# korentomas/mlx-mcmc

Hardware: AMD Instinct MI355X
Metric: leapfrog-steps/sec (all chains) + ESS/sec, 1000-dim Gaussian @1/2/4/8 GPUs (higher is better)
Workload: dtype f32

## Files before the change

### mlx-mcmc_amd/csrc/lanes_fast_nc.h

```cpp
#pragma once
#include "lanes_fast.h"

namespace mc {

template <int NC>
using lf_vec = float __attribute__((ext_vector_type(NC)));
typedef lf_vec<1> f1;
MC_DEV f1 vpin(f1 x) {
    x[0] = vpin((float)x[0]);
    return x;
}
template <int NC>
MC_DEV lf_vec<NC> lf_mk(float a, float b) {
    if constexpr (NC == 2) return (f2){a, b};
    else return (f1){a};
}
template <int NC>
MC_DEV lf_vec<NC> lf_bc(float x) {
    return lf_mk<NC>(x, x);
}
template <class V>
MC_DEV V lf_fma(V a, V b, V c) { return __builtin_elementwise_fma(a, b, c); }
template <int NC>
MC_DEV lf_vec<NC> lf_shc(float v, int k) {
    lf_vec<NC> r;
#pragma unroll
    for (int c = 0; c < NC; ++c) r[c] = rl(v, lf_shlane(k, c));
    return r;
}

template <class V>
struct LfMomV {
    V c, R, R2, Q, n;
};
template <class V>
MC_DEV void lf_moments(const LfMomV<V>& m, V th, V& M1, V& M2) {
    const V d = m.c - th;
    M1 = lf_fma(m.n, d, m.R);
    M2 = lf_fma(lf_fma(m.n, d, m.R2), d, m.Q);
}

constexpr int lfc_draw_jobs(int D, int NC) { return NC * ((D + 3) / 4) + NC; }
constexpr LfDrawJob lfc_draw_job(int t, int D, int NC) {
    const int NBk = (D + 3) / 4;
    const bool acc = t >= NC * NBk;
    const int c = acc ? t - NC * NBk : (t >= NBk ? 1 : 0);
    return {acc, c, acc ? 0 : t - (c ? NBk : 0)};
}
constexpr bool lfc_draw_jobs_once(int D, int lanes, int NC) {
    const int NBk = (D + 3) / 4;
    int mom[2][257] = {}, acc[2] = {};
    if (NBk > 257) return false;
    for (int tid = 0; tid < lanes; ++tid)
        for (int t = tid; t < lfc_draw_jobs(D, NC); t += lanes) {
            const LfDrawJob jb = lfc_draw_job(t, D, NC);
            if (jb.c < 0 || jb.c >= NC || jb.b < 0 || jb.b >= NBk) return false;
            if (jb.acc) ++acc[jb.c];
            else ++mom[jb.c][jb.b];
        }
    for (int c = 0; c < NC; ++c) {
        if (acc[c] != 1) return false;
        for (int b = 0; b < NBk; ++b)
            if (mom[c][b] != 1) return false;
    }
    return true;
}
static_assert(lfc_draw_jobs(1000, 2) == lf_draw_jobs(1000) && lfc_draw_jobs_once(1000, 512, 2) &&
              lfc_draw_job(300, 1000, 2).c == lf_draw_job(300, 1000).c &&
              lfc_draw_job(501, 1000, 2).acc && lf_draw_job(501, 1000).acc,
              "NC = 2: the pair kernel's job map");
static_assert(lfc_draw_jobs(1000, 1) == 251 && lfc_draw_jobs_once(1000, 512, 1) &&
              lfc_draw_jobs_once(1027, 256, 1) && lfc_draw_jobs_once(5, 256, 1) &&
              lfc_draw_jobs_once(303, 256, 1) && lfc_draw_jobs_once(1024, 512, 1),
              "one chain's jobs");

template <int RS, int NSH, int NW, bool X1, int FORM, bool XL = false, int SPEC = 0, int DN = 0,
          int NC = 2>
__global__ void __launch_bounds__(64 * NW)
k_hmc_lfc(LrCtx P, RunArgs A, int64_t chain_base, int64_t n_groups, mc_chain_scalars* scal,
         float* st_q, float* st_g, float* samples, TraceDev tr, unsigned long long* xch,
         int* status, uint32_t ebase) {
    static_assert(NSH <= kLrMaxShared, "shared parameters");
    constexpr bool CF = FORM >= 0;
    static_assert(!CF || lf_nroles(FORM) == NSH, "record slots of a compile-time form");
    constexpr bool DENSE = DN > 0;
    static_assert(!DENSE || (DN == NW && DN >= 2 && DN <= kLrSlices && !X1 && !XL),
                  "dense: wave w is slice w, records through LDS");
    static_assert(DENSE && (NC == 1 || NC == 2), "k_hmc_lfc: the dense launches");
    typedef lf_vec<NC> fc;
    constexpr int NB = DENSE ? NC : 2 * NW;
    constexpr int NV = 2 * (NSH + 1);
    constexpr int NPAIR = NV + 4;
    constexpr int NPASS = (NPAIR + 3) / 4, NPASS_V = (NV + 3) / 4;
    constexpr int NRS = (NV + 7) / 8;
    if (!X1 && !DENSE && A.fault && blockIdx.x == gridDim.x - 1)
        return;
    extern __shared__ __attribute__((aligned(16))) float smem[];
    const mc_run_config& cfg = A.cfg;
    const int tid = threadIdx.x;
    const int wave = tid >> 6, j = tid & 63;
    const int S = DENSE ? DN : P.S, D = P.D, Dsh = P.Dsh;
    int64_t grp;
    int slice;
    if constexpr (DENSE) {
        grp = blockIdx.x;
        slice = wave;
    } else {
        const int64_t w = blockIdx.x, nwg = gridDim.x;
        if (nwg % 8 == 0 && (nwg / 8) % S == 0) {
            const int64_t x = w & 7, r = w >> 3;
            grp = x * ((nwg / 8) / S) + r / S;
            slice = (int)(r % S);
        } else {
            grp = w / S;
            slice = (int)(w % S);
        }
    }
    const int64_t C = cfg.num_chains;
    const int64_t cbase = chain_base + grp * NB;
    const int b0 = DENSE ? 0 : 2 * wave;
    int64_t cc[2];
    bool live[2];
#pragma unroll
    for (int c = 0; c < 2; ++c) {
        live[c] = c < NC && cbase + b0 + c < C;
        cc[c] = min(cbase + b0 + (c < NC ? c : 0), C - 1);
    }

    float* const xl = smem;
    const int64_t* blk = P.blocks + 4 * (int64_t)slice;
    const float* gd = P.data + blk[0];
    const int nsweep = (int)(blk[3] & 255);
    const int ndirect = (int)((blk[3] >> 8) & 255);
    LrSterm* sst = (LrSterm*)(smem + (DENSE ? 2 * DN * 16 : 0));
    for (int i = tid; i < P.n_sterms * (int)(sizeof(LrSterm) / 16); i += 64 * NW)
        ((float4*)sst)[i] = ((const float4*)P.sterms)[i];

    const MC_CONST LrTerm* tt = cptr(P.terms) + (int64_t)slice * P.n_terms;
    const LfTerms F = lf_terms(tt, nsweep, ndirect);
    const bool SW = CF ? (FORM & LF_SW) != 0 : F.sw;
    const bool SWS = CF ? (FORM & LF_SWS) != 0 : F.sw_shs;
    const bool DIR = CF ? (FORM & LF_DIR) != 0 : F.dir;
    const bool DM = CF ? (FORM & LF_DM) != 0 : F.d_shm;
    const bool DS = CF ? (FORM & LF_DS) != 0 : F.d_shs;
    const int ksw = CF ? lf_slot_sws(FORM) : max(F.sw_ks, 0);
    const int kdm = CF ? lf_slot_dm(FORM) : max(F.d_km, 0);
    const int kds = CF ? lf_slot_ds(FORM) : max(F.d_ks, 0);
    const int nsl = CF ? NSH : Dsh;
    auto ord_of = [&](int k) {
        int o = F.d_ks;
        o = (DM && k == kdm) ? F.d_km : o;
        o = (SWS && k == ksw) ? F.sw_ks : o;
        return CF ? o : k;
    };
    int xk = -1, xc = 0;
#pragma unroll
    for (int k = 0; k < kLrMaxShared; ++k)
#pragma unroll
        for (int c = 0; c < NC; ++c)
            if (k < nsl && lf_shlane(k, c) == j) {
                xk = k;
                xc = c;
            }
    const bool xon = xk >= 0;
    const int xo = xon ? ord_of(xk) : 0;
    int xg = P.shl[0];
#pragma unroll
    for (int k = 1; k < kLrMaxShared; ++k) xg = (xo == k) ? P.shl[k] : xg;
    const int64_t xch_id = xc ? cc[1] : cc[0];
    const bool xlive = xon && (xc ? live[1] : live[0]);
    const int rep = (SPEC & LFS_REP1) ? 1 : P.rep;
    const bool lead = (j & (rep - 1)) == 0;
    const bool hxf = (SPEC & LFS_NOXF) ? false : P.has_xf != 0;
    int xxf = P.shxf[0];
    float xid = P.shid[0];
#pragma unroll
    for (int k = 1; k < kLrMaxShared; ++k) {
        xxf = (xo == k) ? P.shxf[k] : xxf;
        xid = (xo == k) ? P.shid[k] : xid;
    }
    xxf = xon ? xxf : MC_XF_NONE;
    xid = xon ? xid : 0.0f;

    LrPriv<RS> R0;
    int gk[RS];
    fc q[RS], p[RS], g[RS];
#pragma unroll
    for (int r = 0; r < RS; ++r) {
        gk[r] = P.gidx[((int64_t)slice * kLrMaxSlots + r) * 64 + j];
#pragma unroll
        for (int c = 0; c < 2; ++c) {
            R0.q[r][c] = gk[r] >= 0 ? st_q[cc[c] * D + gk[r]] : 0.0f;
            R0.g[r][c] = gk[r] >= 0 ? st_g[cc[c] * D + gk[r]] : 0.0f;
        }
        q[r] = lf_mk<NC>(R0.q[r][0], R0.q[r][1]);
        g[r] = lf_mk<NC>(R0.g[r][0], R0.g[r][1]);
        p[r] = lf_bc<NC>(0.0f);
    }
    const bool rngp = P.rng != nullptr;
    int4 rw = {0, 0, 0, 0};
    if (rngp) rw = P.rng[(int64_t)slice * 64 + j];
    const int racc0 = __builtin_amdgcn_readfirstlane((rw.w >> 8) & 63);
    const int racc1 = __builtin_amdgcn_readfirstlane((rw.w >> 14) & 63);
    int sh_src = 0;
    if (rngp) {
        const int target = (xc + 1) | ((xg >> 2) << 3);
        for (int i = 0; i < 64; ++i)
            sh_src = (__builtin_amdgcn_readlane(rw.x, i) == target) ? i : sh_src;
    }
    LrShared sh;
    sh.q = xon ? st_q[xch_id * D + xg] : 1.0f;
    sh.g = xon ? st_g[xch_id * D + xg] : 0.0f;
    sh.p = 0.0f;
    sh.v = hxf ? xf_apply(xxf, sh.q) : sh.q;
    sh.is = sh.iv = 1.0f;
    sh.lg = 0.0f;
    double eps[2];
    fc lp;
    int nacc[2], ntot[2], wacc[2], wtot[2];
#pragma unroll
    for (int c = 0; c < NC; ++c) {
        eps[c] = scal[cc[c]].step_size;
        lp[c] = scal[cc[c]].logp;
        nacc[c] = scal[cc[c]].n_accept;
        ntot[c] = scal[cc[c]].n_total;
        wacc[c] = scal[cc[c]].warmup_accept;
        wtot[c] = scal[cc[c]].warmup_total;
    }
    constexpr bool BDRAW = (DENSE || (X1 && RS == 4)) &&
                           FORM == (LF_SW | LF_SWS | LF_DIR | LF_DM | LF_DS) &&
                           SPEC == (LFS_REP1 | LFS_NOXF);
    const bool bdraw = BDRAW && P.blk_rng != 0;
    const int NBk = (D + 3) >> 2;
    const int ZB = 4 * NC * NBk + 4;
    static_assert(sizeof(LrSterm) % 16 == 0, "the draws' float4 stores follow the scalar terms");
    float* const zl = (float*)sst + P.n_sterms * (int)(sizeof(LrSterm) / 4);
    auto draw_block = [&](int64_t itd) {
        float* const zb = zl + (int)(itd & 1) * ZB;
        for (int t = tid; t < lfc_draw_jobs(D, NC); t += 64 * NW) {
            const LfDrawJob jb = lfc_draw_job(t, D, NC);
            const bool acl = jb.acc;
            const int c = jb.c, b = jb.b;
            const mc_u32x4 rr =
                mc_draw(cfg.seed, (uint32_t)(cfg.chain_offset + (c ? cc[1] : cc[0])),
                        (uint32_t)itd, acl ? MC_RNG_TAG_ACCEPT : MC_RNG_TAG_MOMENTUM, 0,
                        acl ? 0u : (uint32_t)b);
            const float la = mc_logf_unit(acl ? mc_u01_f32(rr.x) : mc_u01_boxf(rr.x));
            const float lb = mc_logf_unit(mc_u01_boxf(rr.z));
            float4 z;
            mc_box_muller_log(la, rr.y, &z.x, &z.y);
            mc_box_muller_log(lb, rr.w, &z.z, &z.w);
            if (acl) zb[4 * NC * NBk + c] = la;
            else *(float4*)(zb + 4 * (c * NBk + b)) = z;
        }
    };
    if constexpr (BDRAW) {
        if (bdraw && cfg.iter_count > 0) draw_block(cfg.iter_begin);
    }
    MC_STAMP_INIT
    __syncthreads();

    const LrOwn own = lr_own_prior(P.n_sterms, sst, xon ? 2 * xo + xc : 64, Dsh);
    const bool own_lp0 = own.on && slice == 0 && xc == 0;
    const bool own_lp1 = own.on && slice == 0 && xc == 1;
    const float o_m = vpin(own.hn ? 0.0f : own.m), o_cinv2 = vpin(own.cinv2),
                o_c0l = vpin(own.c0l), o_wn = vpin(own.wn);
    auto own_grad = [&](float v) {
        const float d = v - o_m;
        const bool out = own.hn && !(v >= 0.0f);
        return (out || !own.on) ? 0.0f : o_wn * -(d * o_cinv2);
    };
    int len[RS];
    fc cnt[RS];
    LfMomV<fc> mom[RS];
    bool pdir[RS];
#pragma unroll
    for (int r = 0; r < RS; ++r) {
        float4 m = {0.f, 0.f, 0.f, 0.f};
        if (SW && r < tt[0].nslot) m = P.mom[((int64_t)slice * kLrMaxSlots + r) * 64 + j];
        len[r] = (int)m.w;
        cnt[r] = lf_bc<NC>(m.w);
        mom[r].c = vpin(lf_bc<NC>(m.x));
        mom[r].R = vpin(lf_bc<NC>(m.y));
        mom[r].R2 = vpin(lf_bc<NC>(m.y + m.y));
        mom[r].Q = vpin(lf_bc<NC>(m.z));
        mom[r].n = cnt[r];
        pdir[r] = DIR && r < tt[nsweep].nslot &&
                  ((const int32_t*)gd)[tt[nsweep].len_off + r * 64 + j] > 0;
    }
    const fc sw_w = vpin(lf_bc<NC>(F.sw_w)), sw_c0 = vpin(lf_bc<NC>(F.sw_c0));
    const fc sw_cinv = vpin(lf_bc<NC>(F.sw_cinv)), sw_cinv2 = vpin(lf_bc<NC>(F.sw_cinv2)),
             sw_clogs = vpin(lf_bc<NC>(F.sw_clogs));
    const fc d_w = vpin(lf_bc<NC>(F.d_w)), d_c0 = vpin(lf_bc<NC>(F.d_c0)), d_m = vpin(lf_bc<NC>(F.d_m));
    const fc d_w1 = vpin(lf_bc<NC>(pdir[0] ? F.d_w : 0.0f));
    const fc d_cinv = vpin(lf_bc<NC>(F.d_cinv)), d_cinv2 = vpin(lf_bc<NC>(F.d_cinv2)),
             d_clogs = vpin(lf_bc<NC>(F.d_clogs));
    const fc half = lf_bc<NC>(0.5f), one = lf_bc<NC>(1.0f);
    const float lp_const = vpin(P.lp_const);
    const int L = cfg.num_leapfrog_steps;
    uint32_t epoch = ebase;
    bool ok = true;
    unsigned long long* gline[2];
#pragma unroll
    for (int par = 0; par < 2; ++par)
        gline[par] = DENSE ? nullptr
                           : xch + (((int64_t)par * n_groups + grp) * (NB / 2) + wave) * S * 16;
    const int row = j >> 4, col = j & 15;
    const bool poll_lane = col < S;
    unsigned long long* gp[2];
#pragma unroll
    for (int par = 0; par < 2; ++par)
        gp[par] = DENSE ? nullptr : gline[par] + min(col, S - 1) * 16 + lf_row(row);
    const int lpoll = min(col, S - 1) * 16 + lf_row(row);
    auto lput = [&](int par, int off, float v) { xl[par * (DN * 16) + off] = v; };
    const int pub_pair = (col < 2 * NRS) ? 8 * (col >> 1) + 4 * (col & 1) + lf_row(row) : -1;
    const bool pub_rec = pub_pair >= 0 && pub_pair < NV && (NC == 2 || !(pub_pair & 1));
    const bool pub_mid = pub_rec && pub_pair >= 2;
    const int pub_x = 2 * (col >> 1) + (col & 1);
    const int pub_off = slice * 16 + max(pub_pair, 0);
    uint32_t need_v = 0, need_lp = 0, need_k0 = 0, need_k1 = 0;
#pragma unroll
    for (int ps = 0; ps < NPASS; ++ps) {
        const int pr = 4 * ps + lf_row(row);
        if (X1 || !poll_lane || pr >= NPAIR || (NC == 1 && (pr & 1))) continue;
        if (pr < 2) need_lp |= 1u << ps;
        else if (pr < NV) need_v |= 1u << ps;
        else if (pr < NV + 2) need_k0 |= 1u << ps;
        else need_k1 |= 1u << ps;
    }
    constexpr bool xchk = XL && !X1;
    unsigned long long* const xslots = xch + ((int64_t)grp * (NB / 2)) * S * 16 + 15;
    XcdPoll xpoll = {0ull};
    if (xchk && cfg.iter_count > 0)
        xpoll = xcd_announce(xslots, S, slice, ebase + 1, wave == 0 && j == 0);
    static_assert(NPAIR <= 15, "granule 15 of a record line is the XCD handshake's");
    const int64_t it_end = cfg.iter_begin + cfg.iter_count;
    constexpr bool DRAW_AHEAD = RS == 1 && CF && (SPEC & LFS_REP1) != 0;
    fc nx_z[RS];
    float nx_sh = 0.0f, nx_lu[2] = {0.f, 0.f};
#pragma unroll
    for (int r = 0; r < RS; ++r) nx_z[r] = lf_bc<NC>(0.0f);
    auto draw_plan = [&](int64_t itd) {
        const int kind = rw.x & 7;
        const bool acl = kind >= 3;
        const int csel = (kind == 2 || kind == 4) ? 1 : 0;
        const mc_u32x4 rr =
            mc_draw(cfg.seed, (uint32_t)(cfg.chain_offset + (csel ? cc[1] : cc[0])),
                    (uint32_t)itd, acl ? MC_RNG_TAG_ACCEPT : MC_RNG_TAG_MOMENTUM, 0,
                    acl ? 0u : ((uint32_t)rw.x >> 3));
        const float la = mc_logf_unit(acl ? mc_u01_f32(rr.x) : mc_u01_boxf(rr.x));
        const float lb = mc_logf_unit(mc_u01_boxf(rr.z));
        float z[4];
        mc_box_muller_log(la, rr.y, &z[0], &z[1]);
        mc_box_muller_log(lb, rr.w, &z[2], &z[3]);
        nx_lu[0] = rl(la, racc0);
        nx_lu[1] = rl(la, racc1);
        auto fetch = [&](int src, int comp) {
            float v = __shfl(z[0], src);
            const float v1 = __shfl(z[1], src), v2 = __shfl(z[2], src), v3 = __shfl(z[3], src);
            v = comp == 1 ? v1 : v;
            v = comp == 2 ? v2 : v;
            return comp == 3 ? v3 : v;
        };
#pragma unroll
        for (int r = 0; r < RS; ++r) {
            const int word = (r < 2 ? rw.y : rw.z) >> (14 * (r & 1));
            const int comp = (word >> 12) & 3;
            nx_z[r] = lf_mk<NC>(fetch(word & 63, comp), fetch((word >> 6) & 63, comp));
        }
        nx_sh = fetch(sh_src, xg & 3);
    };
    if (DRAW_AHEAD && rngp && cfg.iter_count > 0) draw_plan(cfg.iter_begin);
    for (int64_t it = cfg.iter_begin; it < it_end && ok; ++it) {
        MC_STAMP_DECL
        const bool warm = it < cfg.num_warmup;
        float hs[2], es[2];
#pragma unroll
        for (int c = 0; c < NC; ++c) {
            if (it == cfg.num_warmup) {
                wacc[c] = nacc[c];
                wtot[c] = ntot[c];
                nacc[c] = 0;
                ntot[c] = 0;
            }
            hs[c] = (float)(0.5 * eps[c]);
            es[c] = (float)eps[c];
        }
        if constexpr (NC == 1) {
            hs[1] = hs[0];
            es[1] = es[0];
        }
        const fc h = vpin(lf_mk<NC>(hs[0], hs[1])), e = vpin(lf_mk<NC>(es[0], es[1]));
        const float xh = vpin(xc ? hs[1] : hs[0]), xe = vpin(xc ? es[1] : es[0]);
        auto normal_of = [&](int gi, int64_t chain) {
            const mc_u32x4 rr = mc_draw(cfg.seed, (uint32_t)(cfg.chain_offset + chain),
                                        (uint32_t)it, MC_RNG_TAG_MOMENTUM, 0, (uint32_t)(gi >> 2));
            float z0, z1;
            if ((gi & 3) < 2) mc_box_muller(rr.x, rr.y, &z0, &z1);
            else mc_box_muller(rr.z, rr.w, &z0, &z1);
            return (gi & 1) ? z1 : z0;
        };
        fc k0p = lf_bc<NC>(0.0f);
        float logu_acc[2] = {0.f, 0.f};
        if (rngp) {
            if constexpr (DRAW_AHEAD) {
                logu_acc[0] = nx_lu[0];
                logu_acc[1] = nx_lu[1];
#pragma unroll
                for (int r = 0; r < RS; ++r) {
                    if (gk[r] < 0) continue;
                    p[r] = nx_z[r];
                    if (lead) k0p += nx_z[r] * nx_z[r];
                }
                sh.p = xon ? nx_sh : 0.0f;
            } else {
                const int kind = rw.x & 7;
                const bool acl = kind >= 3;
                const int csel = (kind == 2 || kind == 4) ? 1 : 0;
                const mc_u32x4 rr =
                    mc_draw(cfg.seed, (uint32_t)(cfg.chain_offset + (csel ? cc[1] : cc[0])),
                            (uint32_t)it, acl ? MC_RNG_TAG_ACCEPT : MC_RNG_TAG_MOMENTUM, 0,
                            acl ? 0u : ((uint32_t)rw.x >> 3));
                const float la = mc_logf_unit(acl ? mc_u01_f32(rr.x) : mc_u01_boxf(rr.x));
                const float lb = mc_logf_unit(mc_u01_boxf(rr.z));
                float z[4];
                mc_box_muller_log(la, rr.y, &z[0], &z[1]);
                mc_box_muller_log(lb, rr.w, &z[2], &z[3]);
                logu_acc[0] = rl(la, racc0);
                logu_acc[1] = rl(la, racc1);
                auto fetch = [&](int src, int comp) {
                    float v = __shfl(z[0], src);
                    const float v1 = __shfl(z[1], src), v2 = __shfl(z[2], src), v3 = __shfl(z[3], src);
                    v = comp == 1 ? v1 : v;
                    v = comp == 2 ? v2 : v;
                    return comp == 3 ? v3 : v;
                };
    #pragma unroll
                for (int r = 0; r < RS; ++r) {
                    const int word = (r < 2 ? rw.y : rw.z) >> (14 * (r & 1));
                    const int comp = (word >> 12) & 3;
                    const fc zz = lf_mk<NC>(fetch(word & 63, comp), fetch((word >> 6) & 63, comp));
                    if (gk[r] < 0) continue;
                    p[r] = zz;
                    if (lead) k0p += zz * zz;
                }
                const float zs = fetch(sh_src, xg & 3);
                sh.p = xon ? zs : 0.0f;
            }
        } else if (bdraw) {
            if constexpr (X1) __syncthreads();
            const float* const zb = zl + (int)(it & 1) * ZB;
#pragma unroll
            for (int c = 0; c < NC; ++c) logu_acc[c] = zb[4 * NC * NBk + c];
#pragma unroll
            for (int r = 0; r < RS; ++r) {
                const int gi = max(gk[r], 0);
                fc z;
#pragma unroll
                for (int c = 0; c < NC; ++c) z[c] = zb[4 * NBk * c + gi];
                if (gk[r] >= 0) {
                    p[r] = z;
                    if (lead) k0p += z * z;
                }
            }
            const float zs = zb[(xc ? 4 * NBk : 0) + xg];
            sh.p = xon ? zs : 0.0f;
        } else {
#pragma unroll
            for (int r = 0; r < RS; ++r) {
                if (gk[r] < 0) continue;
                fc z;
#pragma unroll
                for (int c = 0; c < NC; ++c) z[c] = normal_of(gk[r], cc[c]);
                p[r] = z;
                if (lead) k0p += z * z;
            }
            sh.p = xon ? normal_of(xg, xch_id) : 0.0f;
        }
        const float K0w[2] = {wave_sum(k0p[0]), wave_sum(k0p[NC - 1])};
        float k0s[2] = {0.f, 0.f};
        {
            const float p2 = sh.p * sh.p;
            for (int k = 0; k < nsl; ++k) {
#pragma unroll
                for (int c = 0; c < NC; ++c) k0s[c] += lf_sh(p2, k, c);
            }
        }
        fc q0[RS], g0[RS];
#pragma unroll
        for (int r = 0; r < RS; ++r) {
            q0[r] = q[r];
            g0[r] = g[r];
        }
        const float q0s = sh.q, g0s = sh.g;
        fc lpn = lp;
        float K0[2] = {0.f, 0.f}, K1[2] = {0.f, 0.f};
        MC_STAMP(5);
        auto drift_private = [&](bool second_half) {
#pragma unroll
            for (int r = 0; r < RS; ++r) {
                const fc hg = h * g[r];
                fc pj = p[r];
                if (second_half) pj = pj + hg;
                pj = pj + hg;
                p[r] = pj;
                q[r] = q[r] + e * pj;
            }
        };
        float gown = 0.0f;
        auto drift_shared = [&](bool second_half) {
            const float hg = xh * sh.g;
            float pj = sh.p;
            if (second_half) pj = pj + hg;
            pj = pj + hg;
            sh.p = pj;
            sh.q = sh.q + xe * pj;
            sh.v = sh.q;
            if (hxf) sh.v = xf_apply(xxf, sh.q);
            sh.is = __builtin_amdgcn_rcpf(sh.v);
            sh.iv = sh.is * sh.is;
            gown = vpin(own_grad(sh.v));
        };
        drift_private(false);
        drift_shared(false);
        if (xchk && it == cfg.iter_begin) {
            const bool same = xcd_agree(xpoll, xslots, S, ebase + 1, ok);
            if (ok && slice == 0 && wave == 0 && j == 0)
                __hip_atomic_fetch_add(status + (same ? 8 : 9), 1, __ATOMIC_RELAXED,
                                       __HIP_MEMORY_SCOPE_AGENT);
            if (!ok || !same) {
                __hip_atomic_store(status, ok ? 2 : 1, __ATOMIC_RELAXED, __HIP_MEMORY_SCOPE_AGENT);
                ok = false;
                break;
            }
        }
        auto step = [&](int l, auto kind, auto parc, auto& ahead) -> bool {
            constexpr int KIND = decltype(kind)::value;
            constexpr int PAR = decltype(parc)::value;
            constexpr bool FIRST = KIND == 0 || KIND == 3, LAST = KIND == 2 || KIND == 3;
            (void)l;
            if constexpr (!DENSE)
                __builtin_amdgcn_s_waitcnt(0x0F70);
            if constexpr (LAST)
                sh.lg = __builtin_amdgcn_logf(sh.v) * 0.693147180559945f;
            MC_STAMP(0);
            constexpr bool lst = LAST;
            const fc z0 = lf_bc<NC>(0.0f);
            fc lpp = z0, cs = z0, cm = z0, cd = z0;
            bool lpp0 = true, cs0 = true, cm0 = true, cd0 = true;
            bool g0r[RS];
#pragma unroll
            for (int r = 0; r < RS; ++r) {
                g[r] = lf_bc<NC>(0.0f);
                g0r[r] = true;
            }
            auto acc = [](fc& s, bool& first, fc v) {
                s = first ? v : s + v;
                first = false;
            };
            fc M2[RS];
            if (SW) {
                const fc is = SWS ? lf_shc<NC>(sh.is, ksw) : sw_cinv;
                const fc iv = SWS ? is * is : sw_cinv2;
#pragma unroll
                for (int r = 0; r < RS; ++r) {
                    const bool on = len[r] != 0;
                    const fc z = lf_bc<NC>(0.0f);
                    fc m1, m2;
                    lf_moments(mom[r], q[r], m1, m2);
                    const fc M1r = on ? m1 : z;
                    M2[r] = on ? m2 : z;
                    if (RS == 1) {
                        g[r] = sw_w * (M1r * iv);
                        cs = sw_w * ((M2[r] * iv - cnt[r]) * is);
                        cs0 = g0r[r] = false;
                    } else if (on) {
                        acc(g[r], g0r[r], sw_w * (M1r * iv));
                        acc(cs, cs0, sw_w * ((M2[r] * iv - cnt[r]) * is));
                    }
                    if (lst) {
                        const fc lg = SWS ? lf_shc<NC>(sh.lg, ksw) : sw_clogs;
                        const fc lpt = cnt[r] * (sw_c0 - lg) - (half * M2[r]) * iv;
                        if (RS == 1) {
                            lpp = on ? sw_w * lpt : z;
                            lpp0 = false;
                        } else if (on) {
                            acc(lpp, lpp0, sw_w * lpt);
                        }
                    }
                }
            }
            if (DIR) {
                const fc um = DM ? lf_shc<NC>(sh.v, kdm) : d_m;
                const fc is = DS ? lf_shc<NC>(sh.is, kds) : d_cinv;
                const fc iv = DS ? is * is : d_cinv2;
#pragma unroll
                for (int r = 0; r < RS; ++r) {
                    if (RS > 1 && !pdir[r]) continue;
                    const fc dw = RS == 1 ? d_w1 : d_w;
                    const fc d = q[r] - um;
                    const fc s2 = d * d;
                    const fc u = dw * (d * iv);
                    acc(g[r], g0r[r], -u);
                    acc(cm, cm0, u);
                    acc(cd, cd0, dw * ((s2 * iv - one) * is));
                    if (lst) {
                        const fc lg = DS ? lf_shc<NC>(sh.lg, kds) : d_clogs;
                        const fc lpt = one * (d_c0 - lg) - (half * s2) * iv;
                        acc(lpp, lpp0, dw * lpt);
                    }
                }
            }
            static_assert(NC == 2 || (SPEC & LFS_REP1) != 0, "one chain per wave: rep == 1");
            static_assert(NC == 2 || (SPEC & LFS_NOXF) != 0, "one chain per wave: no transform");
            if constexpr (NC == 2) {
                if (rep > 1) {
#pragma unroll
                    for (int r = 0; r < RS; ++r) {
                        float a = g[r][0], b = g[r][1];
                        grp_sum2(a, b, rep);
                        g[r] = (fc){a, b};
                    }
                }
            }
            const float g_own = gown;
            {
                if (lst) {
                    const float v = sh.v;
                    const float d = v - o_m;
                    const bool out = own.hn && !(v >= 0.0f);
                    const float d2 = d * d;
                    const float lpe = out ? -__builtin_inff() : o_c0l - (0.5f * d2) * o_cinv2;
                    const float lp_own = o_wn * lpe;
                    if constexpr (NC == 2) {
                        if (own_lp0) lpp[0] += lp_own;
                        if (own_lp1) lpp[1] += lp_own;
                    } else {
                        static_assert(lf_shlane(0, 1) == lf_shlane(0, 0) + 32 &&
                                      lf_shlane(1, 1) == lf_shlane(1, 0) + 32 &&
                                      lf_shlane(2, 1) == lf_shlane(2, 0) + 32 &&
                                      lf_shlane(3, 1) == lf_shlane(3, 0) + 32, "chain 1's holders");
                        const bool odd = (cbase & 1) != 0;
                        const float lp_up = __shfl_xor(own_lp0 ? lp_own : 0.0f, 32);
                        const bool on_up = __shfl_xor(own_lp0 ? 1 : 0, 32) != 0;
                        if (odd ? on_up : own_lp0) lpp[0] += odd ? lp_up : lp_own;
                    }
                    if (hxf && slice == 0 && xon) {
                        if (xc == 0) lpp[0] += xid * sh.q;
                        else if constexpr (NC == 2) lpp[1] += xid * sh.q;
                    }
                }
            }
            MC_STAMP(1);
            float xr[2 * NRS];
            {
                float v[8 * NRS];
#pragma unroll
                for (int x = 0; x < 8 * NRS; ++x) v[x] = 0.0f;
#pragma unroll
                for (int c = 0; c < NC; ++c) v[c] = lpp[c];
                if constexpr (CF) {
#pragma unroll
                    for (int c = 0; c < NC; ++c) {
                        if (FORM & LF_SWS) v[2 + 2 * lf_slot_sws(FORM) + c] = cs[c];
                        if (FORM & LF_DM) v[2 + 2 * lf_slot_dm(FORM) + c] = cm[c];
                        if (FORM & LF_DS) v[2 + 2 * lf_slot_ds(FORM) + c] = cd[c];
                    }
                } else {
#pragma unroll
                    for (int k = 0; k < NSH; ++k)
#pragma unroll
                        for (int c = 0; c < NC; ++c)
                            v[2 + 2 * k + c] = ((F.sw_ks == k ? cs[c] : 0.0f) +
                                                (F.d_km == k ? cm[c] : 0.0f)) +
                                               (F.d_ks == k ? cd[c] : 0.0f);
                }
#pragma unroll
                for (int qq = 0; qq < NRS; ++qq) {
                    float vv[8], xx[2];
#pragma unroll
                    for (int x = 0; x < 8; ++x) vv[x] = v[8 * qq + x];
                    if (qq == 0 && !lst) lf_rs8<true>(vv, xx);
                    else lf_rs8(vv, xx);
                    xr[2 * qq] = xx[0];
                    xr[2 * qq + 1] = xx[1];
                }
            }
            float k1w[2] = {0.f, 0.f};
            if constexpr (LAST) {
                fc k1p = lf_bc<NC>(0.0f);
#pragma unroll
                for (int r = 0; r < RS; ++r) {
                    const fc pj = p[r] + h * g[r];
                    if (lead) k1p += pj * pj;
                }
#pragma unroll
                for (int c = 0; c < NC; ++c) k1w[c] = wave_sum(k1p[c]);
            }
            ++epoch;
            const int par = PAR >= 0 ? PAR : (int)(epoch & 1);
            if constexpr (!X1 && !FIRST && !LAST) {
                float pv = xr[0];
#pragma unroll
                for (int x = 1; x < 2 * NRS; ++x) pv = (x == pub_x) ? xr[x] : pv;
                if constexpr (DENSE) {
                    if (pub_mid) lput(par, pub_off, pv);
                } else {
                    if (pub_mid) granule_put(gline[par] + pub_off, epoch, pv, XL);
                }
            } else if (!X1) {
                int pp = -1;
                float pv = 0.0f;
                if (pub_rec && (lst || pub_pair >= 2)) {
                    pp = pub_pair;
                    pv = xr[0];
#pragma unroll
                    for (int x = 1; x < 2 * NRS; ++x)
                        if (x == 2 * (col >> 1) + (col & 1)) pv = xr[x];
                }
                if (col == 2 * NRS || (NC == 2 && col == 2 * NRS + 1)) {
                    const int c = col - 2 * NRS;
                    if (FIRST && row == 0) {
                        pp = NV + c;
                        pv = c ? K0w[1] : K0w[0];
                    }
                    if (LAST && row == 1) {
                        pp = NV + 2 + c;
                        pv = c ? k1w[1] : k1w[0];
                    }
                }
                if constexpr (DENSE) {
                    if (pp >= 0) lput(par, slice * 16 + pp, pv);
                } else {
                    if (pp >= 0) granule_put(gline[par] + slice * 16 + pp, epoch, pv, XL);
                }
            }
            MC_STAMP(2);
            if constexpr (!DENSE) __builtin_amdgcn_s_setprio(1);
            constexpr bool kstep = FIRST || LAST;
            const uint32_t need =
                need_v | (FIRST ? need_k0 : 0u) | (LAST ? (need_k1 | need_lp) : 0u);
            float vals[NPASS];
#pragma unroll
            for (int ps = 0; ps < NPASS; ++ps) vals[ps] = 0.0f;
            unsigned long long y[NPASS];
            auto poll_issue = [&]() {
#pragma unroll
                for (int ps = 0; ps < NPASS; ++ps)
                    y[ps] = (ps < NPASS_V || kstep) ? granule_load(gp[par] + 4 * ps) : 0ull;
            };
            if constexpr (!LAST) drift_private(true);
            if constexpr (LAST) ahead();
            MC_STAMP(8);
            if (!X1 && !DENSE) poll_issue();
            auto poll_eval = [&]() {
                bool ready = true;
#pragma unroll
                for (int ps = 0; ps < NPASS; ++ps) {
                    const bool nd = ((need >> ps) & 1u) != 0u;
                    vals[ps] = nd ? __uint_as_float((uint32_t)y[ps]) : 0.0f;
                    ready = ready & (!nd | ((uint32_t)(y[ps] >> 32) == epoch));
                }
                return ready;
            };
            if constexpr (DENSE) {
                __syncthreads();
#pragma unroll
                for (int ps = 0; ps < NPASS; ++ps) {
                    const bool nd = ((need >> ps) & 1u) != 0u;
                    const float v = (ps < NPASS_V || kstep) ? xl[par * (DN * 16) + lpoll + 4 * ps] : 0.0f;
                    vals[ps] = nd ? v : 0.0f;
                }
            }
            if constexpr (!DENSE) {
                bool ready = X1 ? true : poll_eval();
                MC_STAMP(7);
                uint32_t spins = 0;
                while (__ballot(!ready)) {
                    if (++spins > kSpinLimit) {
                        ok = false;
                        break;
                    }
                    poll_issue();
                    ready = poll_eval();
                }
                if (__builtin_expect(!ok, 0)) return false;
            } else {
                MC_STAMP(7);
            }
            MC_STAMP(3);
            if constexpr (!DENSE) __builtin_amdgcn_s_setprio(0);
            float tot[NPASS];
            if constexpr (X1) {
#pragma unroll
                for (int ps = 0; ps < NPASS; ++ps) tot[ps] = ps < 2 * NRS ? xr[ps] : 0.0f;
            } else {
#pragma unroll
                for (int ps = 0; ps < NPASS; ++ps) {
                    float t = vals[ps];
                    if (ps < NPASS_V || kstep) {
                        t += lf_dpp<0xB1>(t);
                        t += lf_dpp<0x4E>(t);
                        t += lf_dpp<0x141>(t);
                        t += lf_dpp<0x140>(t);
                    }
                    tot[ps] = t;
                }
            }
            if constexpr (LAST) {
#pragma unroll
                for (int c = 0; c < NC; ++c) lpn[c] = rl(tot[0], 16 * lf_row(c)) + lp_const;
            }
            {
                float gx = 0.0f;
#pragma unroll
                for (int ps = 0; ps < NPASS_V; ++ps)
                    if (col == ps) gx = tot[ps];
                float gt = gx + g_own;
                if (hxf) gt = xf_chain(xxf, gt, sh.q, sh.v) + xid;
                sh.g = xon ? gt : 0.0f;
            }
            if constexpr (FIRST) {
                constexpr int p0 = NV, p1 = NV + 1;
                if constexpr (X1) {
                    K0[0] = K0w[0];
                    K0[1] = K0w[1];
                } else {
                    K0[0] = rl(tot[p0 / 4], 16 * lf_row(p0));
                    if constexpr (NC == 2) K0[1] = rl(tot[p1 / 4], 16 * lf_row(p1));
                }
            }
            if constexpr (LAST) {
                constexpr int p0 = NV + 2, p1 = NV + 3;
                if constexpr (X1) {
                    K1[0] = k1w[0];
                    K1[1] = k1w[1];
                } else {
                    K1[0] = rl(tot[p0 / 4], 16 * lf_row(p0));
                    if constexpr (NC == 2) K1[1] = rl(tot[p1 / 4], 16 * lf_row(p1));
                }
            }
            if constexpr (!LAST) drift_shared(true);
            MC_STAMP(4);
            return true;
        };
        auto draw_next = [&]() {
            if constexpr (DRAW_AHEAD) {
                if (rngp && it + 1 < it_end) draw_plan(it + 1);
            }
            if constexpr (BDRAW) {
                if (bdraw && it + 1 < it_end) draw_block(it + 1);
            }
        };
        const std::integral_constant<int, -1> rtpar;
        if (L == 1) {
            ok = step(0, std::integral_constant<int, 3>(), rtpar, draw_next);
        } else {
            ok = step(0, std::integral_constant<int, 0>(), rtpar, draw_next);
            const std::integral_constant<int, 1> mid;
            if (X1) {
                for (int l = 1; ok && l < L - 1; ++l) ok = step(l, mid, rtpar, draw_next);
            } else {
                const std::integral_constant<int, 0> par0;
                const std::integral_constant<int, 1> par1;
                int n = L - 2;
                if (n > 0 && !(epoch & 1)) {
                    ok = step(1, mid, par1, draw_next);
                    --n;
                }
                for (; __builtin_expect(ok, 1) && n >= 2; n -= 2) {
                    ok = step(1, mid, par0, draw_next);
                    if (__builtin_expect(ok, 1)) ok = step(1, mid, par1, draw_next);
                }
                if (ok && n == 1) ok = step(1, mid, par0, draw_next);
            }
            if (ok) ok = step(L - 1, std::integral_constant<int, 2>(), rtpar, draw_next);
        }
        if (!ok) {
            __hip_atomic_store(status, 1, __ATOMIC_RELAXED, __HIP_MEMORY_SCOPE_AGENT);
            break;
        }
        float k1s[2] = {0.f, 0.f};
        {
            const float p1 = sh.p + xh * sh.g;
            const float p2 = p1 * p1;
            for (int k = 0; k < nsl; ++k) {
#pragma unroll
                for (int c = 0; c < NC; ++c) k1s[c] += lf_sh(p2, k, c);
            }
        }
        bool acc[2];
        if constexpr (NC == 1) acc[1] = false;
#pragma unroll
        for (int c = 0; c < NC; ++c) {
            const float H0 = -lp[c] + 0.5f * (K0[c] + k0s[c]);
            const float H1 = -lpn[c] + 0.5f * (K1[c] + k1s[c]);
            const float ratio = -(H1 - H0);
            float logu = logu_acc[c];
            if (!rngp && !bdraw) {
                const mc_u32x4 ru = mc_draw(cfg.seed, (uint32_t)(cfg.chain_offset + cc[c]),
                                            (uint32_t)it, MC_RNG_TAG_ACCEPT, 0, 0);
                logu = mc_logf_u01(mc_u01_f32(ru.x));
            }
            const bool accepted = logu < ratio;
            acc[c] = accepted;
            nacc[c] += accepted ? 1 : 0;
            ntot[c] += 1;
            const double eps_used = eps[c];
            if (warm && cfg.adapt_step_size && it > 10) {
                const double rate = (double)nacc[c] / (double)ntot[c];
                eps[c] = (rate < cfg.target_accept) ? eps_used * 0.95 : eps_used * 1.05;
            }
            if (accepted) lp[c] = lpn[c];
            if (slice == 0 && j == 0 && live[c]) {
                const int64_t ti = it - tr.iter_begin;
                if (ti >= 0 && ti < tr.capacity) {
                    const int64_t o = cc[c] * tr.capacity + ti;
                    if (tr.accepted) tr.accepted[o] = accepted ? 1 : 0;
                    if (tr.accept_stat) tr.accept_stat[o] = ratio;
                    if (tr.step_size) tr.step_size[o] = eps_used;
                    if (tr.energy) tr.energy[o] = H0;
                    if (tr.tree_depth) tr.tree_depth[o] = L;
                    if (tr.n_leapfrog) tr.n_leapfrog[o] = L;
                }
            }
        }
#pragma unroll
        for (int r = 0; r < RS; ++r) {
            q[r] = lf_mk<NC>(acc[0] ? q[r][0] : q0[r][0],
                             acc[NC - 1] ? q[r][NC - 1] : q0[r][NC - 1]);
            g[r] = lf_mk<NC>(acc[0] ? g[r][0] : g0[r][0],
                             acc[NC - 1] ? g[r][NC - 1] : g0[r][NC - 1]);
        }
        if (!(xc ? acc[1] : acc[0])) {
            sh.q = q0s;
            sh.g = g0s;
        }
        if (!warm && samples != nullptr) {
            const int64_t s = it - cfg.num_warmup - cfg.sample_begin;
            if (s >= 0 && s < cfg.sample_capacity) {
#pragma unroll
                for (int c = 0; c < NC; ++c) {
                    if (!live[c]) continue;
                    float* out = samples + (cc[c] * cfg.sample_capacity + s) * (int64_t)D;
#pragma unroll
                    for (int r = 0; r < RS; ++r)
                        if (gk[r] >= 0 && lead) out[gk[r]] = q[r][c];
                }
                if (slice == 0 && xlive)
                    samples[(xch_id * cfg.sample_capacity + s) * (int64_t)D + xg] = sh.q;
            }
        }
        MC_STAMP(6);
    }

    MC_STAMP_FLUSH
    if (!ok) return;
#pragma unroll
    for (int c = 0; c < NC; ++c) {
        if (!live[c]) continue;
#pragma unroll
        for (int r = 0; r < RS; ++r) {
            if (gk[r] >= 0 && lead) {
                st_q[cc[c] * D + gk[r]] = q[r][c];
                st_g[cc[c] * D + gk[r]] = g[r][c];
            }
        }
        if (slice == 0 && j == 0) {
            mc_chain_scalars& sc = scal[cc[c]];
            sc.logp = lp[c];
            sc.step_size = eps[c];
            sc.n_accept = nacc[c];
            sc.n_total = ntot[c];
            sc.warmup_accept = wacc[c];
            sc.warmup_total = wtot[c];
            sc.n_grad += cfg.iter_count * (int64_t)L;
        }
    }
    if (slice == 0 && xlive) {
        st_q[xch_id * D + xg] = sh.q;
        st_g[xch_id * D + xg] = sh.g;
    }
}


}
```

### mlx-mcmc_amd/csrc/run_lanes.h

```cpp
#pragma once
#include "launch.h"
#include "lanes_fast_nc.h"

template <int NW, bool X1, typename K>
inline int hmc_lr_exchange(const char* name, K& k, const mc_program* p, const mc_run_config* cfg,
                           void* state, float* samples, const mc_trace* tr, void* ws,
                           hipStream_t st, bool fast = false) {
    RunState R = run_state(p, cfg, state);
    const LrCtx ctx = lrctx_of(p);
    const TraceDev td = trace_of(tr);
    constexpr int NB = 2 * NW;
    ExchangeLaunch d;
    d.name = name;
    d.threads = 64 * NW;
    d.chains = NB;
    d.S = p->lr.S;
    d.lds = fast ? p->lr.sterms.size() * sizeof(LrSterm) : lr_base_lds_bytes(p);
    d.blocks_per_launch = lr_groups_per_launch(p, cfg->num_chains);
    d.clear_bytes = sl_workspace_bytes(p, cfg->num_chains);
    d.tags_per_launch = (uint64_t)cfg->iter_count * cfg->num_leapfrog_steps + 1;
    d.restart_tags = false;
    d.coresident = !X1;
    int* status = (int*)ws;
    unsigned long long* xch = (unsigned long long*)((char*)ws + kSlStatusBytes);
    return run_exchange(d, k, cfg->num_chains, ws, st, R.A,
                        [&](int64_t g0, int64_t ng, int64_t grid, bool xl, uint32_t base) {
        return k.launch(xl, grid, d.threads, d.lds, st, ctx, R.A, g0 * NB, ng, R.scalars, R.q, R.g,
                        samples, td, xch, status, base);
    });
}

template <int RS, int NSH, int NW, bool X1>
inline int launch_hmc_lr(const mc_program* p, const mc_run_config* cfg, void* state,
                         float* samples, const mc_trace* tr, void* ws, hipStream_t st) {
    if (p->lr.has_expr) {
        ModulePair k{p, "mc::k_hmc_lr<" + std::to_string(RS) + ", " + std::to_string(NSH) + ", " +
                            std::to_string(NW) + ", " + (X1 ? "true" : "false")};
        const int rc = k.load();
        if (rc != MC_OK) return rc;
        if (k.f == nullptr) return kLanesNoJit;
        return hmc_lr_exchange<NW, X1>("lane-resident HMC (expression JIT)", k, p, cfg, state,
                                       samples, tr, ws, st);
    }
    const bool fast = p->lr.fast && lanes_fast_enabled();
    auto kern = fast ? k_hmc_lf<RS, NSH, NW, X1, -1> : k_hmc_lr<RS, NSH, NW, X1>;
    auto kern_xl = (fast || X1) ? kern : k_hmc_lr<RS, NSH, NW, X1, true>;
    const bool forms = lanes_forms_enabled();
    if constexpr (NSH == 3) {
        constexpr int HIER = LF_SW | LF_SWS | LF_DIR | LF_DM | LF_DS;
        if (fast && forms && p->lr.form == HIER) {
            kern = k_hmc_lf<RS, lf_nroles(HIER), NW, X1, HIER>;
            kern_xl = X1 ? kern : k_hmc_lf<RS, lf_nroles(HIER), NW, X1, HIER, true>;
            if constexpr (RS == 1) {
                constexpr int PLAIN = LFS_REP1 | LFS_NOXF;
                if (p->lr.rep == 1 && p->lr.has_xf == 0) {
                    kern = k_hmc_lf<RS, lf_nroles(HIER), NW, X1, HIER, false, PLAIN>;
                    kern_xl =
                        X1 ? kern : k_hmc_lf<RS, lf_nroles(HIER), NW, X1, HIER, true, PLAIN>;
                }
            }
        }
        if (fast && forms && p->lr.form == LF_DIR) {
            kern = k_hmc_lf<RS, lf_nroles(LF_DIR), NW, X1, LF_DIR>;
            kern_xl = X1 ? kern : k_hmc_lf<RS, lf_nroles(LF_DIR), NW, X1, LF_DIR, true>;
        }
    }
    auto k = static_pair(kern, kern_xl);
    return hmc_lr_exchange<NW, X1>("lane-resident HMC", k, p, cfg, state, samples, tr, ws, st,
                                   fast);
}

template <int RS>
inline int launch_hmc_dense(const mc_program* p, const mc_run_config* cfg, void* state,
                            float* samples, const mc_trace* tr, void* ws, hipStream_t st) {
    constexpr int HIER = LF_SW | LF_SWS | LF_DIR | LF_DM | LF_DS;
    constexpr int PLAIN = LFS_REP1 | LFS_NOXF;
    constexpr int NSH = lf_nroles(HIER);
    const LanePlan& L = p->lrd;
    RunState R = run_state(p, cfg, state);
    const LrCtx ctx = lrctx_of(p, L);
    const TraceDev td = trace_of(tr);
    ws_forget(ws);
    const int nc = L.S == 1 ? 2 : hmc_dense_chains(cfg->num_chains, device_cus(), L.dense_chains);
    const int64_t groups = (cfg->num_chains + nc - 1) / nc;
    const size_t sterm_bytes = L.sterms.size() * sizeof(LrSterm);
    const size_t draw_bytes =
        L.blk_rng ? (size_t)2 * (4 * nc * ((p->D + 3) / 4) + 4) * 4 : 0;
    auto go = [&](auto kern, int waves) {
        const size_t lds =
            sterm_bytes + draw_bytes + (waves > 1 ? (size_t)2 * waves * 16 * 4 : 0);
        hipLaunchKernelGGL(kern, dim3((unsigned)groups), dim3(64 * waves), lds, st, ctx, R.A,
                           (int64_t)0, groups, R.scalars, R.q, R.g, samples, td,
                           (unsigned long long*)nullptr, (int*)nullptr, (uint32_t)0);
        MC_HIP_TRY(hipGetLastError());
        return MC_OK;
    };
    if (L.S == 1) return go(k_hmc_lf<RS, NSH, 1, true, HIER, false, PLAIN>, 1);
    if constexpr (RS == 2) {
        if (L.S == 4)
            return nc == 1 ? go(k_hmc_lfc<2, NSH, 4, false, HIER, false, PLAIN, 4, 1>, 4)
                           : go(k_hmc_lf<2, NSH, 4, false, HIER, false, PLAIN, 4>, 4);
        if (L.S == 8)
            return nc == 1 ? go(k_hmc_lfc<2, NSH, 8, false, HIER, false, PLAIN, 8, 1>, 8)
                           : go(k_hmc_lf<2, NSH, 8, false, HIER, false, PLAIN, 8>, 8);
    }
    return fail(MC_ERR_UNSUPPORTED, "dense HMC: no kernel for %d slices at %d slots", L.S, RS);
}

template <int RS>
inline int hmc_lanes_dispatch(const mc_program* p, const mc_run_config* cfg, void* state,
                              float* samples, const mc_trace* tr, void* ws, hipStream_t st) {
    const bool w4 = lr_nw(p) == 4, x1 = p->lr.S == 1;
    return dispatch_nsh(p, [&](auto N) {
        constexpr int NSH = decltype(N)::value;
        return x1 ? launch_hmc_lr<RS, NSH, 1, true>(p, cfg, state, samples, tr, ws, st)
             : w4 ? launch_hmc_lr<RS, NSH, 4, false>(p, cfg, state, samples, tr, ws, st)
                  : launch_hmc_lr<RS, NSH, 8, false>(p, cfg, state, samples, tr, ws, st);
    });
}
```

Before: 426.8 million.

## Compact one-chain dense exchange record to four values with permlane reduction

For the one-chain-per-wave dense kernel, the per-step cross-wave record is packed into four values (log p and three shared cotangents) and reduced with permlane32/permlane16 swaps plus DPP instead of the generic 8-per-slot path. The LDS exchange line shrinks from 16*DN to 6*DN floats, each wave reads a single slot and does a shorter reduction, and the own-gradient computation moves after the barrier. The aim is less LDS traffic and fewer cross-lane ops on the critical path of every leapfrog step. It adds complex lane-mapping logic, guarded by constexpr static checks.

```diff
diff --git a/mlx-mcmc_amd/csrc/lanes_fast_nc.h b/mlx-mcmc_amd/csrc/lanes_fast_nc.h
--- a/mlx-mcmc_amd/csrc/lanes_fast_nc.h
+++ b/mlx-mcmc_amd/csrc/lanes_fast_nc.h
@@ -21,11 +21,87 @@
 }
 template <class V>
 MC_DEV V lf_fma(V a, V b, V c) { return __builtin_elementwise_fma(a, b, c); }
+
+constexpr int lfc_rs4_input(int v) { return v == 1 ? 2 : (v == 2 ? 1 : v); }
+constexpr int lfc_rs4_row_input(int r) { return 2 * (r & 1) + (r >> 1); }
+constexpr int lfc_holder(int k) { return 16 * (k + 1); }
+constexpr int lfc_line_floats(int NC, int DN) { return NC == 1 ? 6 * DN : 16 * DN; }
+constexpr int lfc_pub_off(int DN, int slice, int v) { return (void)DN, 4 * slice + v; }
+constexpr int lfc_read_off(int DN, int lane) {
+    const int row = lane >> 4, col = lane & 15;
+    return 4 * (col < DN ? col : DN - 1) + row;
+}
+constexpr bool lfc_rs4_model(int DN, int NSH) {
+    int w[2][64] = {}, t[64] = {};
+    for (int m = 0; m < 2; ++m)
+        for (int l = 0; l < 64; ++l) w[m][l] = 2 * m + (l >= 32 ? 1 : 0);
+    for (int l = 0; l < 64; ++l)
+        t[l] = w[(l >> 4) & 1][32 * (l >> 5)];
+    for (int v = 0; v < 4; ++v) {
+        int rows = 0;
+        for (int r = 0; r < 4; ++r) {
+            for (int c = 1; c < 16; ++c)
+                if (t[16 * r + c] != t[16 * r]) return false;
+            if (t[16 * r] != lfc_rs4_row_input(r)) return false;
+            if (t[16 * r] == lfc_rs4_input(v)) {
+                ++rows;
+                if (r != v) return false;
+            }
+        }
+        if (rows != 1) return false;
+    }
+    for (int s = 0; s < DN; ++s)
+        for (int v = 0; v < 4; ++v) {
+            const int off = lfc_pub_off(DN, s, v);
+            if (off < 0 || off >= 4 * DN) return false;
+            int readers = 0;
+            for (int l = 0; l < 64; ++l)
+                if ((l & 15) < DN && lfc_read_off(DN, l) == off) {
+                    ++readers;
+                    if ((l >> 4) != v || (l & 15) != s) return false;
+                }
+            if (readers != 1) return false;
+        }
+    for (int l = 0; l < 64; ++l)
+        if (lfc_read_off(DN, l) < 0 || lfc_read_off(DN, l) >= 4 * DN) return false;
+    if (4 * DN + 2 * DN != lfc_line_floats(1, DN)) return false;
+    if (NSH > 3) return false;
+    for (int k = 0; k < NSH; ++k) {
+        if (lfc_holder(k) < 0 || lfc_holder(k) >= 64 || (lfc_holder(k) >> 4) != 1 + k) return false;
+        for (int k2 = 0; k2 < k; ++k2)
+            if (lfc_holder(k2) == lfc_holder(k) || lf_shlane(k2, 0) == lf_shlane(k, 0)) return false;
+    }
+    return true;
+}
+static_assert(lfc_rs4_model(8, 3) && lfc_rs4_model(4, 3) && lfc_rs4_model(2, 3) &&
+              lfc_rs4_model(16, 3), "the four-value record's lane maps");
+template <bool Z0 = false>
+MC_DEV float lf_rs4(const float (&v)[4]) {
+    const auto r1 = __builtin_amdgcn_permlane32_swap(__float_as_uint(v[1]), __float_as_uint(v[3]),
+                                                     false, false);
+    const float w1 = __uint_as_float(r1[0]) + __uint_as_float(r1[1]);
+    const auto r0 = __builtin_amdgcn_permlane32_swap(Z0 ? r1[0] : __float_as_uint(v[0]),
+                                                     __float_as_uint(v[2]), false, false);
+    const float w0 = __uint_as_float(r0[0]) + __uint_as_float(r0[1]);
+    const auto r = __builtin_amdgcn_permlane16_swap(__float_as_uint(w0), __float_as_uint(w1),
+                                                    false, false);
+    float t = __uint_as_float(r[0]) + __uint_as_float(r[1]);
+    t += lf_dpp<0xB1>(t);
+    t += lf_dpp<0x4E>(t);
+    t += lf_dpp<0x141>(t);
+    t += lf_dpp<0x140>(t);
+    return t;
+}
+
+template <int NC>
+MC_DEV constexpr int lfc_shlane(int k, int c) {
+    return NC == 1 ? lfc_holder(k) : lf_shlane(k, c);
+}
 template <int NC>
 MC_DEV lf_vec<NC> lf_shc(float v, int k) {
     lf_vec<NC> r;
 #pragma unroll
-    for (int c = 0; c < NC; ++c) r[c] = rl(v, lf_shlane(k, c));
+    for (int c = 0; c < NC; ++c) r[c] = rl(v, lfc_shlane<NC>(k, c));
     return r;
 }
 
@@ -127,12 +203,17 @@
         cc[c] = min(cbase + b0 + (c < NC ? c : 0), C - 1);
     }
 
+    constexpr bool RS4 = NC == 1;
+    static_assert(!RS4 || (CF && NSH == 3 && lfc_rs4_model(DN, NSH)),
+                  "one chain per wave: log p and three cotangents");
+    constexpr int LW = lfc_line_floats(NC, DN);
+    static_assert((2 * LW) % 4 == 0, "the scalar terms' float4 copies follow the lines");
     float* const xl = smem;
     const int64_t* blk = P.blocks + 4 * (int64_t)slice;
     const float* gd = P.data + blk[0];
     const int nsweep = (int)(blk[3] & 255);
     const int ndirect = (int)((blk[3] >> 8) & 255);
-    LrSterm* sst = (LrSterm*)(smem + (DENSE ? 2 * DN * 16 : 0));
+    LrSterm* sst = (LrSterm*)(smem + (DENSE ? 2 * LW : 0));
     for (int i = tid; i < P.n_sterms * (int)(sizeof(LrSterm) / 16); i += 64 * NW)
         ((float4*)sst)[i] = ((const float4*)P.sterms)[i];
 
@@ -158,7 +239,7 @@
     for (int k = 0; k < kLrMaxShared; ++k)
 #pragma unroll
         for (int c = 0; c < NC; ++c)
-            if (k < nsl && lf_shlane(k, c) == j) {
+            if (k < nsl && lfc_shlane<NC>(k, c) == j) {
                 xk = k;
                 xc = c;
             }
@@ -312,7 +393,11 @@
     for (int par = 0; par < 2; ++par)
         gp[par] = DENSE ? nullptr : gline[par] + min(col, S - 1) * 16 + lf_row(row);
     const int lpoll = min(col, S - 1) * 16 + lf_row(row);
-    auto lput = [&](int par, int off, float v) { xl[par * (DN * 16) + off] = v; };
+    auto lput = [&](int par, int off, float v) { xl[par * LW + off] = v; };
+    const int pub4_off = lfc_pub_off(DN, slice, row);
+    const bool pub4 = col == 0, pub4_mid = col == 0 && row > 0;
+    const int lrd4 = lfc_read_off(DN > 0 ? DN : 1, j);
+    const int lrdk = 4 * DN + (row & 1) * DN + min(col, S - 1);
     const int pub_pair = (col < 2 * NRS) ? 8 * (col >> 1) + 4 * (col & 1) + lf_row(row) : -1;
     const bool pub_rec = pub_pair >= 0 && pub_pair < NV && (NC == 2 || !(pub_pair & 1));
     const bool pub_mid = pub_rec && pub_pair >= 2;
@@ -483,7 +568,7 @@
             const float p2 = sh.p * sh.p;
             for (int k = 0; k < nsl; ++k) {
 #pragma unroll
-                for (int c = 0; c < NC; ++c) k0s[c] += lf_sh(p2, k, c);
+                for (int c = 0; c < NC; ++c) k0s[c] += rl(p2, lfc_shlane<NC>(k, c));
             }
         }
         fc q0[RS], g0[RS];
@@ -519,7 +604,7 @@
             if (hxf) sh.v = xf_apply(xxf, sh.q);
             sh.is = __builtin_amdgcn_rcpf(sh.v);
             sh.iv = sh.is * sh.is;
-            gown = vpin(own_grad(sh.v));
+            if constexpr (!RS4) gown = vpin(own_grad(sh.v));
         };
         drift_private(false);
         drift_shared(false);
@@ -623,7 +708,7 @@
                     }
                 }
             }
-            const float g_own = gown;
+            float g_own = gown;
             {
                 if (lst) {
                     const float v = sh.v;
@@ -641,9 +726,14 @@
                                       lf_shlane(2, 1) == lf_shlane(2, 0) + 32 &&
                                       lf_shlane(3, 1) == lf_shlane(3, 0) + 32, "chain 1's holders");
                         const bool odd = (cbase & 1) != 0;
-                        const float lp_up = __shfl_xor(own_lp0 ? lp_own : 0.0f, 32);
-                        const bool on_up = __shfl_xor(own_lp0 ? 1 : 0, 32) != 0;
-                        if (odd ? on_up : own_lp0) lpp[0] += odd ? lp_up : lp_own;
+                        const float lpo = own_lp0 ? lp_own : 0.0f;
+#pragma unroll
+                        for (int k = 0; k < NSH; ++k) {
+                            const float lpk = rl(lpo, lfc_holder(k));
+                            const bool onk =
+                                __builtin_amdgcn_readlane(own_lp0 ? 1 : 0, lfc_holder(k)) != 0;
+                            if (onk && j == lf_shlane(k, 0) + (odd ? 32 : 0)) lpp[0] += lpk;
+                        }
                     }
                     if (hxf && slice == 0 && xon) {
                         if (xc == 0) lpp[0] += xid * sh.q;
@@ -653,7 +743,17 @@
             }
             MC_STAMP(1);
             float xr[2 * NRS];
-            {
+            float xr4 = 0.0f;
+            if constexpr (RS4) {
+                float v[4];
+                v[0] = lpp[0];
+                v[1 + lf_slot_sws(FORM)] = (FORM & LF_SWS) ? cs[0] : 0.0f;
+                v[1 + lf_slot_dm(FORM)] = (FORM & LF_DM) ? cm[0] : 0.0f;
+                v[1 + lf_slot_ds(FORM)] = (FORM & LF_DS) ? cd[0] : 0.0f;
+                xr4 = lst ? lf_rs4(v) : lf_rs4<true>(v);
+#pragma unroll
+                for (int x = 0; x < 2 * NRS; ++x) xr[x] = 0.0f;
+            } else {
                 float v[8 * NRS];
 #pragma unroll
                 for (int x = 0; x < 8 * NRS; ++x) v[x] = 0.0f;
@@ -699,7 +799,23 @@
             }
             ++epoch;
             const int par = PAR >= 0 ? PAR : (int)(epoch & 1);
-            if constexpr (!X1 && !FIRST && !LAST) {
+            if constexpr (RS4 && !FIRST && !LAST) {
+                if (pub4_mid) lput(par, pub4_off, xr4);
+            } else if constexpr (RS4) {
+                int po = (pub4 && (lst || row > 0)) ? pub4_off : -1;
+                float pv = xr4;
+                if (col == 1) {
+                    if (FIRST && row == 0) {
+                        po = 4 * DN + slice;
+                        pv = K0w[0];
+                    }
+                    if (LAST && row == 1) {
+                        po = 5 * DN + slice;
+                        pv = k1w[0];
+                    }
+                }
+                if (po >= 0) lput(par, po, pv);
+            } else if constexpr (!X1 && !FIRST && !LAST) {
                 float pv = xr[0];
 #pragma unroll
                 for (int x = 1; x < 2 * NRS; ++x) pv = (x == pub_x) ? xr[x] : pv;
@@ -765,11 +881,21 @@
             };
             if constexpr (DENSE) {
                 __syncthreads();
-#pragma unroll
-                for (int ps = 0; ps < NPASS; ++ps) {
-                    const bool nd = ((need >> ps) & 1u) != 0u;
-                    const float v = (ps < NPASS_V || kstep) ? xl[par * (DN * 16) + lpoll + 4 * ps] : 0.0f;
-                    vals[ps] = nd ? v : 0.0f;
+                if constexpr (RS4) {
+                    const float va = xl[par * LW + lrd4];
+                    const float vk = kstep ? xl[par * LW + lrdk] : 0.0f;
+                    g_own = own_grad(vpin(sh.v));
+                    vals[0] = poll_lane ? va : 0.0f;
+                    const bool ndk = poll_lane && ((FIRST && row == 0) || (LAST && row == 1));
+                    if constexpr (NPASS > 1) vals[1] = ndk ? vk : 0.0f;
+                } else {
+#pragma unroll
+                    for (int ps = 0; ps < NPASS; ++ps) {
+                        const bool nd = ((need >> ps) & 1u) != 0u;
+                        const float v =
+                            (ps < NPASS_V || kstep) ? xl[par * LW + lpoll + 4 * ps] : 0.0f;
+                        vals[ps] = nd ? v : 0.0f;
+                    }
                 }
             }
             if constexpr (!DENSE) {
@@ -794,6 +920,18 @@
             if constexpr (X1) {
 #pragma unroll
                 for (int ps = 0; ps < NPASS; ++ps) tot[ps] = ps < 2 * NRS ? xr[ps] : 0.0f;
+            } else if constexpr (RS4) {
+#pragma unroll
+                for (int ps = 0; ps < NPASS; ++ps) {
+                    float t = ps < 2 ? vals[ps] : 0.0f;
+                    if (ps == 0 || (ps == 1 && kstep)) {
+                        t += lf_dpp<0xB1>(t);
+                        t += lf_dpp<0x4E>(t);
+                        t += lf_dpp<0x141>(t);
+                        t += lf_dpp<0x140>(t);
+                    }
+                    tot[ps] = t;
+                }
             } else {
 #pragma unroll
                 for (int ps = 0; ps < NPASS; ++ps) {
@@ -813,9 +951,13 @@
             }
             {
                 float gx = 0.0f;
-#pragma unroll
-                for (int ps = 0; ps < NPASS_V; ++ps)
-                    if (col == ps) gx = tot[ps];
+                if constexpr (RS4) {
+                    gx = tot[0];
+                } else {
+#pragma unroll
+                    for (int ps = 0; ps < NPASS_V; ++ps)
+                        if (col == ps) gx = tot[ps];
+                }
                 float gt = gx + g_own;
                 if (hxf) gt = xf_chain(xxf, gt, sh.q, sh.v) + xid;
                 sh.g = xon ? gt : 0.0f;
@@ -825,6 +967,8 @@
                 if constexpr (X1) {
                     K0[0] = K0w[0];
                     K0[1] = K0w[1];
+                } else if constexpr (RS4) {
+                    K0[0] = rl(tot[1], 0);
                 } else {
                     K0[0] = rl(tot[p0 / 4], 16 * lf_row(p0));
                     if constexpr (NC == 2) K0[1] = rl(tot[p1 / 4], 16 * lf_row(p1));
@@ -835,6 +979,8 @@
                 if constexpr (X1) {
                     K1[0] = k1w[0];
                     K1[1] = k1w[1];
+                } else if constexpr (RS4) {
+                    K1[0] = rl(tot[1], 16);
                 } else {
                     K1[0] = rl(tot[p0 / 4], 16 * lf_row(p0));
                     if constexpr (NC == 2) K1[1] = rl(tot[p1 / 4], 16 * lf_row(p1));
@@ -886,7 +1032,7 @@
             const float p2 = p1 * p1;
             for (int k = 0; k < nsl; ++k) {
 #pragma unroll
-                for (int c = 0; c < NC; ++c) k1s[c] += lf_sh(p2, k, c);
+                for (int c = 0; c < NC; ++c) k1s[c] += rl(p2, lfc_shlane<NC>(k, c));
             }
         }
         bool acc[2];
diff --git a/mlx-mcmc_amd/csrc/run_lanes.h b/mlx-mcmc_amd/csrc/run_lanes.h
--- a/mlx-mcmc_amd/csrc/run_lanes.h
+++ b/mlx-mcmc_amd/csrc/run_lanes.h
@@ -87,8 +87,8 @@
     const size_t draw_bytes =
         L.blk_rng ? (size_t)2 * (4 * nc * ((p->D + 3) / 4) + 4) * 4 : 0;
     auto go = [&](auto kern, int waves) {
-        const size_t lds =
-            sterm_bytes + draw_bytes + (waves > 1 ? (size_t)2 * waves * 16 * 4 : 0);
+        const size_t lds = sterm_bytes + draw_bytes +
+                           (waves > 1 ? (size_t)2 * lfc_line_floats(nc, waves) * 4 : 0);
         hipLaunchKernelGGL(kern, dim3((unsigned)groups), dim3(64 * waves), lds, st, ctx, R.A,
                            (int64_t)0, groups, R.scalars, R.q, R.g, samples, td,
                            (unsigned long long*)nullptr, (int*)nullptr, (uint32_t)0);
```

Result: faster. 475.5 million (median of 6 runs) (+11.4%).
